# African-Robotics-Unit/AcinoSet

Measured on AMD Instinct MI355X. Metric: FTE frames/sec (residual+Jac+LM step), 6-cam x 20-joint, higher is better.
Workload: dtype f64

## Files before the change

acinoset_amd/csrc/chunk.hip:

```cpp
#include "chunk.hpp"

#include <algorithm>
#include <cstdlib>

#include "bcr_dev.hpp"
#include "trio80.hpp"

namespace acino {

void ChunkPlan::build(int nodes_total, int chunk_nodes, bool pin_l, bool pin_r) {
  n_nodes = nodes_total;
  m = n_chunks = n_sep = 0;
  node0 = pin_l ? 1 : 0;
  pin_right = pin_r ? 1 : 0;
  const int nodes = nodes_total - node0;
  if (chunk_nodes < 0 || nodes < 1) return;
  int mm = chunk_nodes;
  if (mm == 0) {
    mm = (nodes + 255) / 256;
    mm = std::max(4, std::min(mm, 512));
  }
  mm = std::max(2, mm);
  m = mm;
  n_chunks = (nodes + mm - 1) / mm;
  if (pin_r && n_chunks > 1 && nodes - (n_chunks - 1) * mm == 1) --n_chunks;
  n_sep = n_chunks - 1 + node0 + pin_right;
}

__device__ __forceinline__ d4 tile_u_ut(const double* X, int ib, int jb, int li, int lk) {
  const double* pa = X + (ib * 16 + li) * LD + ib * 16 + lk;
  const double* pb = X + (jb * 16 + li) * LD + ib * 16 + lk;
  const d4 z = {0, 0, 0, 0};
  switch (ib) {
    case 0: return mma_seq<20, false>(z, pa, 4, pb, 4);
    case 1: return mma_seq<16, false>(z, pa, 4, pb, 4);
    case 2: return mma_seq<12, false>(z, pa, 4, pb, 4);
    case 3: return mma_seq<8, false>(z, pa, 4, pb, 4);
    default: return mma_seq<4, false>(z, pa, 4, pb, 4);
  }
}
__device__ __forceinline__ void tile_store(double* M, int ib, int jb, const d4& a, int li, int lk) {
#pragma unroll
  for (int rr = 0; rr < 4; ++rr) M[(ib * 16 + lk + 4 * rr) * LD + jb * 16 + li] = a[rr];
}

constexpr int SW_VEC = 18 * NP + 2 * BS + 8 + 8 + 3 * NP + 64;
static constexpr size_t kSweepLds = (3 * MAT + SW_VEC) * sizeof(double);

__device__ __forceinline__ int opaque(int x) {
  asm volatile("" : "+v"(x));
  return x;
}

constexpr int SW_T = 512;
template <int NQ>
__device__ __forceinline__ void syrk_mask_n(d4 (&acc)[NQ], bool load) {
#pragma unroll
  for (int q = 0; q < NQ; ++q)
#pragma unroll
    for (int rr = 0; rr < 4; ++rr) acc[q][rr] = load ? acc[q][rr] : 0.0;
}
constexpr int SP_STEPS = 4 * NT - 1;
__device__ __forceinline__ void spike_gf(const double* G, const double (&bF)[NT][4], d4 (&acc)[NT], int li, int lk) {
  double a[3][NT];
  const double* gb = G + lk * LD + li;
  auto fetch = [&](int buf, int step) {
#pragma unroll
    for (int ib = 0; ib < NT; ++ib) a[buf][ib] = gb[(4 * step) * LD + ib * 16];
  };
#pragma unroll
  for (int ib = 0; ib < NT; ++ib) acc[ib] = d4{0, 0, 0, 0};
  fetch(0, 0);
  fetch(1, 1);
#pragma unroll
  for (int step = 0; step < SP_STEPS; ++step) {
    if (step + 2 < SP_STEPS) fetch((step + 2) % 3, step + 2);
    __builtin_amdgcn_sched_barrier(0);
#pragma unroll
    for (int ib = 0; ib < NT; ++ib) acc[ib] = mfma(a[step % 3][ib], bF[step >> 2][step & 3], acc[ib]);
    __builtin_amdgcn_sched_barrier(0);
  }
}
template <int NQ>
__device__ __forceinline__ void spike_ftt(d4 (&acc)[NQ], const double* Yf, const d4 (&T)[NT], const int (&as)[NQ], int li, int lk) {
  constexpr int DEPTH = NQ >= 3 ? 2 : (NQ == 2 ? 3 : 6);
  const double* p = Yf + lk * LD + li;
  double a[DEPTH + 1][NQ];
#pragma unroll
  for (int d = 0; d < DEPTH; ++d)
#pragma unroll
    for (int q = 0; q < NQ; ++q) a[d][q] = p[(4 * d) * LD + as[q] * 16];
#pragma unroll
  for (int st = 0; st < SP_STEPS; ++st) {
    if (st + DEPTH < SP_STEPS) {
#pragma unroll
      for (int q = 0; q < NQ; ++q) a[(st + DEPTH) % (DEPTH + 1)][q] = p[(4 * (st + DEPTH)) * LD + as[q] * 16];
    }
    __builtin_amdgcn_sched_barrier(0);
#pragma unroll
    for (int q = 0; q < NQ; ++q) acc[q] = mfma(-a[st % (DEPTH + 1)][q], T[st >> 2][st & 3], acc[q]);
    __builtin_amdgcn_sched_barrier(0);
  }
}
template <int NQ>
struct AlTiles {
  d4 acc[NQ];
  int as[NQ], j;
  double* Ag;
  __device__ __forceinline__ double* at(int q, int rr, int li, int lk) const {
    return as[q] >= j ? Ag + (size_t)(as[q] * 16 + 4 * rr + lk) * BS + j * 16 + li
                      : Ag + (size_t)(j * 16 + li) * BS + as[q] * 16 + 4 * rr + lk;
  }
  __device__ __forceinline__ void fetch(int li, int lk) {
#pragma unroll
    for (int q = 0; q < NQ; ++q)
#pragma unroll
      for (int rr = 0; rr < 4; ++rr) acc[q][rr] = *at(q, rr, li, lk);
  }
  __device__ __forceinline__ void run(bool load, const double* Yf, const d4 (&T)[NT], int li, int lk) {
    syrk_mask_n<NQ>(acc, load);
    spike_ftt<NQ>(acc, Yf, T, as, li, lk);
#pragma unroll
    for (int q = 0; q < NQ; ++q)
#pragma unroll
      for (int rr = 0; rr < 4; ++rr) *at(q, rr, li, lk) = acc[q][rr];
  }
};
__device__ __forceinline__ int role8(int wave) { return (0x75236410u >> (4 * wave)) & 15; }
struct GramQueue {
  int *open, *ticket, *done;
};
__device__ __forceinline__ void gram_help(const GramQueue& q, const double* Xf, double* Xg, int k, int li, int lk, int lane) {
  for (;;) {
    int t = 0;
    if (lane == 0) t = __hip_atomic_fetch_add(q.ticket, 1, __ATOMIC_RELAXED, __HIP_MEMORY_SCOPE_WORKGROUP);
    t = __builtin_amdgcn_readfirstlane(t) - 15 * k;
    if (t >= 15) {
      if (lane == 0) __hip_atomic_fetch_add(q.ticket, -1, __ATOMIC_RELAXED, __HIP_MEMORY_SCOPE_WORKGROUP);
      return;
    }
    const int ib = tri_i(t), jb = tri_j(t);
    const d4 g = tile_u_ut(Xf, ib, jb, li, lk);
#pragma unroll
    for (int rr = 0; rr < 4; ++rr) {
      Xg[(ib * 16 + lk + 4 * rr) * LD + jb * 16 + li] = g[rr];
      if (ib != jb) Xg[(jb * 16 + li) * LD + ib * 16 + lk + 4 * rr] = g[rr];
    }
    lds_signal(q.done, lane);
  }
}

struct SpikeArgs {
  const double* Xg;
  double* Y;
  double* Ag;
  const double* cRk;
  const double* bvn;
  double* zk;
  int *c_gfdone, *c_fready, *c_bv, *tdone;
  GramQueue gq;
  const double* Xf;
  int k, n_s;
  bool hasL, has_next;
  long long* stamps;
};
template <int ROLE>
__device__ __forceinline__ void spike_node(const SpikeArgs& A, int& tsb, int ln) {
  constexpr bool two = ROLE == 5;
  constexpr int j0 = ROLE == 4 ? 1 : (ROLE == 5 ? 2 : (ROLE == 6 ? 3 : 4));
  constexpr int NA = ROLE == 4 ? 3 : (ROLE == 5 ? 2 : (ROLE == 6 ? 5 : 4));
  const int li = ln & 15, lk = ln >> 4;
  double* const Y = A.Y;
  auto stamp = [&](int i) { if (A.stamps && ln == 0) A.stamps[i] = (long long)wall_clock64(); };
  AlTiles<NA> al;
  AlTiles<1> al0;
  al.Ag = A.Ag;
  al.j = j0;
  if (ROLE == 4) { al.as[0] = 1; al.as[1] = 0; al.as[2 % NA] = 2; }
  if (ROLE == 5) { al.as[0] = 2; al.as[1] = 0; }
  if (ROLE == 6) { al.as[0] = 3; al.as[1] = 0; al.as[2 % NA] = 1; al.as[3 % NA] = 2; al.as[4 % NA] = 4; }
  if (ROLE == 7) { al.as[0] = 4; al.as[1] = 0; al.as[2 % NA] = 1; al.as[3 % NA] = 2; }
  al0.Ag = A.Ag;
  al0.j = 0;
  al0.as[0] = 0;
  if (A.hasL) {
    al.fetch(li, lk);
    if (two) al0.fetch(li, lk);
  }
  lds_wait(A.gq.open, A.k + 1);
  gram_help(A.gq, A.Xf, const_cast<double*>(A.Xg), A.k, li, lk, ln);
  lds_wait(A.gq.done, 15 * (A.k + 1));
  stamp(16 + 4 * (ROLE - 4));
  d4 T0[NT], T1[NT];
  {
    double bF[NT][4];
    const double* yb = Y + lk * LD + j0 * 16 + li;
#pragma unroll
    for (int kb = 0; kb < NT; ++kb)
#pragma unroll
      for (int s = 0; s < 4; ++s) bF[kb][s] = (4 * kb + s < SP_STEPS) ? yb[(kb * 16 + 4 * s) * LD] : 0.0;
    spike_gf(A.Xg, bF, T0, li, lk);
  }
  if (two) {
    double bF[NT][4];
    const double* yb = Y + lk * LD + li;
#pragma unroll
    for (int kb = 0; kb < NT; ++kb)
#pragma unroll
      for (int s = 0; s < 4; ++s) bF[kb][s] = (4 * kb + s < SP_STEPS) ? yb[(kb * 16 + 4 * s) * LD] : 0.0;
    spike_gf(A.Xg, bF, T1, li, lk);
  }
  lds_signal(A.c_gfdone, ln);
  stamp(17 + 4 * (ROLE - 4));
  if (A.hasL) {
    lds_wait(A.c_fready, A.n_s * A.k);
    al.run(A.k > 0, Y, T0, li, lk);
    if (two) al0.run(A.k > 0, Y, T1, li, lk);
  }
  stamp(18 + 4 * (ROLE - 4));
  if (A.hasL) {
    if (ROLE != 5) lds_signal(A.tdone + (ROLE == 4 ? 0 : (ROLE == 6 ? 1 : 2)), ln);
    if (ROLE == 7 || ROLE == 4 || ROLE == 5) lds_wait(A.tdone + 1, A.k + 1);
    if (ROLE == 4 || ROLE == 5) lds_wait(A.tdone + 2, A.k + 1);
    if (ROLE == 5) lds_wait(A.tdone + 0, A.k + 1);
  }
  (void)tsb;
#pragma unroll
  for (int ib = 0; ib < NT; ++ib) tile_store(Y, ib, j0, T0[ib], li, lk);
  if (two) {
#pragma unroll
    for (int ib = 0; ib < NT; ++ib) tile_store(Y, ib, 0, T1[ib], li, lk);
  }
  if (ROLE == 7) {
    A.zk[ln] = Y[ln * LD + (BS - 1)];
    if (ln < 16) A.zk[64 + ln] = Y[(64 + ln) * LD + (BS - 1)];
  }
  if (A.has_next) {
    lds_wait(A.c_bv, A.k + 1);
    const double* const cRk = A.cRk;
    const double* const bvn = A.bvn;
    const int p = ln % NP, cg = ln / NP;
#pragma unroll
    for (int h = 0; h < (two ? 2 : 1); ++h) {
      const int c_lo = 16 * (h ? 0 : j0);
      if (cg < 2) {
        const double e00 = cRk[(0 * 3 + 0) * NP + p], e01 = cRk[(0 * 3 + 1) * NP + p], e02 = cRk[(0 * 3 + 2) * NP + p];
        const double e11 = cRk[(1 * 3 + 1) * NP + p], e12 = cRk[(1 * 3 + 2) * NP + p], e22 = cRk[(2 * 3 + 2) * NP + p];
        const double b0 = bvn[p], b1 = bvn[NP + p], b2 = bvn[2 * NP + p];
        double fv[8][3];
#pragma unroll
        for (int q = 0; q < 8; ++q) {
          const int cc = c_lo + cg + 2 * q;
          fv[q][0] = Y[p * LD + cc];
          fv[q][1] = Y[(NP + p) * LD + cc];
          fv[q][2] = Y[(2 * NP + p) * LD + cc];
        }
#pragma unroll
        for (int q = 0; q < 8; ++q) {
          const int cc = c_lo + cg + 2 * q;
          const double f0 = fv[q][0], f1 = fv[q][1], f2 = fv[q][2];
          double o0 = -(e00 * f0 + e01 * f1 + e02 * f2), o1 = -(e11 * f1 + e12 * f2), o2 = -(e22 * f2);
          if (cc == BS - 1) {
            o0 += b0;
            o1 += b1;
            o2 += b2;
          }
          Y[p * LD + cc] = o0;
          Y[(NP + p) * LD + cc] = o1;
          Y[(2 * NP + p) * LD + cc] = o2;
        }
      }
      if (ln < 16)
        for (int r = 3 * NP; r < BS; ++r) Y[r * LD + c_lo + ln] = 0.0;
    }
  }
  lds_signal(A.c_fready, ln);
  stamp(19 + 4 * (ROLE - 4));
}


__global__ void __launch_bounds__(SW_T)
k_chunk_sweep(BcrChain ch, SepView sp, const FteConst* __restrict__ cst, int* numeric_err, const int* __restrict__ status,
                int m, int n_chunks, int node0, int pin_right) {
  extern __shared__ __attribute__((aligned(16))) char smem_raw[];
  if (status && *status != 0) return;
  double* const Xf = reinterpret_cast<double*>(smem_raw);
  double* const Xg = Xf + MAT;
  double* const Y = Xg + MAT;
  double* const cL = Y + MAT;
  double* const cR0 = cL + 9 * NP;
  double* const bvb = cR0 + 9 * NP;
  double* const red = bvb + 2 * BS;
  int* const sync = reinterpret_cast<int*>(red + 8);
  int* const cB = sync + 5;
  int* const tdone = sync + 2;
  int* const g_done = sync + 6;
  int* const g_open = sync + 10;
  int* const g_ticket = sync + 1;
  int* const c_gfdone = sync + 7;
  int* const c_fready = sync + 8;
  int* const c_bv = sync + 9;
  double* const kq = red + 16;
  double* const klo = kq + NP;
  double* const khi = klo + NP;
  long long* const lst = reinterpret_cast<long long*>(khi + NP);
  const int tid = threadIdx.x, wave = tid >> 6, lane = tid & 63;
  const FteConst& K = *cst;
  const int c = blockIdx.x;
  const int first = node0 + c * m;
  const bool hasL = c > 0 || node0 > 0, hasR = c + 1 < n_chunks || pin_right;
  const int len = c + 1 < n_chunks ? m : ch.n_nodes - first;
  const int n_int = hasR ? len - 1 : len;
  const int sL = c - 1 + node0, sR = c + node0;
  const size_t MB = (size_t)BS * BS;
  const int role = __builtin_amdgcn_readfirstlane(role8(wave));
  const bool uni_tables = coupling_tables_uniform(K, first, first + n_int - 1);
  const int n_s = hasL ? 4 : 1;
  const bool builder = role <= 3;
  const bool strips = role >= 4 && (hasL || role == 7);
  double gmax_run = 0.0;
  long long* const dbgp = (ch.dbg && (long long)blockIdx.x == ch.dbg[64] && ch.dbg[66] == 0) ? ch.dbg : nullptr;
  const int dbg_k = dbgp ? (int)ch.dbg[65] : -1;
  if (dbgp && lane == 0) {
    const unsigned hw = __builtin_amdgcn_s_getreg((31 << 11) | 4);
    atomicOr(reinterpret_cast<unsigned long long*>(ch.dbg + 67), (unsigned long long)((hw >> 4) & 3) << (4 * wave));
    if (wave == 0) ch.dbg[68] = hw;
  }
#define SW_STAMP(i) do { if (dbgp && k == dbg_k && lane == 0) lst[i] = (long long)wall_clock64(); } while (0)
  if (tid < 16) sync[tid] = 0;
  if (tid < 64) lst[tid] = 0;
  if (dbgp && tid == 0) dbgp[70] = (long long)wall_clock64();
  if (c == 0 && node0) {
    for (int e = tid; e < BS * BS; e += SW_T) sp.D[e] = 0.0;
    if (tid < BS) sp.b[tid] = 0.0;
  }
  if (tid < NP) {
    kq[tid] = K.q_w[tid];
    klo[tid] = K.lo[tid];
    khi[tid] = K.hi[tid];
  }
  __syncthreads();

  TrioSync tsy;
  {
    NodeFetch f;
    build_fetch<SW_T>(f, ch, K, first, tid);
    fill_coupling_coef<SW_T>(cL, cR0, K, first, tid, kq);
    for (int e = tid; e < MAT; e += SW_T) Y[e] = 0.0;
    gmax_run = build_finish<SW_T>(Xf, bvb, f, K, first, tid, kq, klo, khi);
    __syncthreads();
    if (dbgp && tid == 0) lst[60] = (long long)wall_clock64();
    if (hasL)
      for (int e = tid; e < 9 * NP; e += SW_T) {
        const int pair = e / NP, p = e % NP, ii = pair / 3, jj = pair % 3;
        if (ii <= jj) Y[(ii * NP + p) * LD + jj * NP + p] = cL[e];
      }
    if (tid < BS) Y[tid * LD + (BS - 1)] = bvb[tid];
    __syncthreads();
    if (role < 3) chol80_trio(Xf, role, lane, numeric_err, sync, tsy);
    __syncthreads();
    if (dbgp && tid == 0) lst[61] = (long long)wall_clock64();
  }

  int tb = 0, tsb = 0;
#pragma unroll 1
  for (int k = 0; k < n_int; ++k) {
    const int node = first + k, next = node + 1;
    const bool last = k + 1 == n_int;
    const bool has_next = !last || hasR;
    const int ln = opaque(lane);
    const int li = ln & 15, lk = ln >> 4;
    double* const cRk = (uni_tables || !(k & 1)) ? cR0 : cL;
    if (builder) {
      const int bw = role;
      const int bt = bw * 64 + ln;
      const int fb_next = 3 * (next - node0);
      double hq[2][3] = {{0, 0, 0}, {0, 0, 0}}, xq[3] = {0, 0, 0}, gq[3] = {0, 0, 0}, cvq[3] = {0, 0, 0}, lamq = 0.0;
      bool liveq[3] = {false, false, false}, ownq[3] = {false, false, false};
      int pdq[2], pcq[2];
      bool ownp[2], dgp[2];
      int pdg = 0;
      bool anydg = false;
#pragma unroll
      for (int sl = 0; sl < 2; ++sl) {
        const int e = bt + 256 * sl;
        ownp[sl] = e < 13 * NP;
        const int pa = ownp[sl] ? e / 13 : 0, dd = ownp[sl] ? e % 13 : 0;
        pdq[sl] = pa;
        pcq[sl] = pa + dd >= NP ? pa + dd - NP : pa + dd;
        dgp[sl] = ownp[sl] && dd == 0;
        if (dgp[sl]) pdg = pa;
        anydg = anydg || dgp[sl];
      }
      if (has_next) {
        const int cur = ch.st->cur;
        const double* Hg = cur ? ch.H1 : ch.H0;
        lamq = ch.st->lam;
#pragma unroll
        for (int j = 0; j < 3; ++j)
          if (fb_next + j < K.n_frames) {
#pragma unroll
            for (int sl = 0; sl < 2; ++sl)
              if (ownp[sl]) hq[sl][j] = Hg[(size_t)(fb_next + j) * HPAIRS + bt + 256 * sl];
          }
        if (anydg) {
          const double* xg = cur ? ch.x1 : ch.x0;
          const double* gg = cur ? ch.g1 : ch.g0;
#pragma unroll
          for (int j = 0; j < 3; ++j)
            if (fb_next + j < K.n_frames) {
              xq[j] = xg[(size_t)(fb_next + j + HALO) * NP + pdg];
              gq[j] = gg[(size_t)(fb_next + j) * NP + pdg];
            }
#pragma unroll
          for (int pr = 0; pr < 3; ++pr) {
            const int j = pr == 2 ? 1 : 0, jp = pr == 0 ? 1 : 2;
            if (fb_next + jp < K.n_frames)
              cvq[pr] = 2.0 * kq[pdg] * band_coef_clip(K.n_offset + fb_next + j, jp - j, K.n_global, K.clip_len);
          }
        }
#pragma unroll
        for (int j = 0; j < 3; ++j) {
          liveq[j] = fb_next + j < K.n_frames;
          ownq[j] = fb_next + j >= K.own_lo && fb_next + j < K.own_hi;
        }
      }
      if (bw == 0) SW_STAMP(0);
      lds_barrier(cB, tb, 4, ln);
      lds_wait(c_gfdone, n_s * k);
      if (bw == 0) SW_STAMP(1);
      const GramQueue gqu{g_open, g_ticket, g_done};
      if (bt == 0) __hip_atomic_fetch_add(g_open, 1, __ATOMIC_RELAXED, __HIP_MEMORY_SCOPE_WORKGROUP);
      if (k > 0 && !uni_tables) fill_coupling_coef<256>(nullptr, cRk, K, node, bt, kq);
      gram_help(gqu, Xf, Xg, k, li, lk, ln);
      SW_STAMP(32 + wave);
      lds_barrier(cB, tb, 4, ln);
      lds_wait(g_done, 15 * (k + 1));
      if (bw == 0) SW_STAMP(2);
#pragma unroll
      for (int j = 0; j < 3; ++j) asm volatile("" : "+v"(hq[0][j]), "+v"(hq[1][j]), "+v"(xq[j]), "+v"(gq[j]));
      asm volatile("" : "+v"(lamq));
      if (has_next) {
        double* const bvn = bvb + ((k + 1) & 1) * BS;
        double ca[2][6], cb[2][6], gv[2][3][3];
#pragma unroll
        for (int sl = 0; sl < 2; ++sl) {
          const int pr = pdq[sl], pc = pcq[sl];
          ca[sl][0] = cRk[0 * NP + pr]; ca[sl][1] = cRk[1 * NP + pr]; ca[sl][2] = cRk[2 * NP + pr];
          ca[sl][3] = cRk[4 * NP + pr]; ca[sl][4] = cRk[5 * NP + pr]; ca[sl][5] = cRk[8 * NP + pr];
          cb[sl][0] = cRk[0 * NP + pc]; cb[sl][1] = cRk[1 * NP + pc]; cb[sl][2] = cRk[2 * NP + pc];
          cb[sl][3] = cRk[4 * NP + pc]; cb[sl][4] = cRk[5 * NP + pc]; cb[sl][5] = cRk[8 * NP + pc];
#pragma unroll
          for (int jj = 0; jj < 3; ++jj) {
            const double* gp = Xg + (jj * NP + pr) * LD + pc;
            gv[sl][jj][0] = gp[0];
            gv[sl][jj][1] = gp[NP];
            gv[sl][jj][2] = gp[2 * NP];
          }
        }
#pragma unroll
        for (int sl = 0; sl < 2; ++sl) {
          const int pr = pdq[sl], pc = pcq[sl];
          const bool dg = dgp[sl];
          const double a00 = ca[sl][0], a01 = ca[sl][1], a02 = ca[sl][2], a11 = ca[sl][3], a12 = ca[sl][4], a22 = ca[sl][5];
          const double b00 = cb[sl][0], b01 = cb[sl][1], b02 = cb[sl][2], b11 = cb[sl][3], b12 = cb[sl][4], b22 = cb[sl][5];
          double mm[3][3], S[3][3];
#pragma unroll
          for (int jj = 0; jj < 3; ++jj) {
            const double g0 = gv[sl][jj][0], g1 = gv[sl][jj][1], g2 = gv[sl][jj][2];
            mm[jj][0] = g0 * b00 + g1 * b01 + g2 * b02;
            mm[jj][1] = g1 * b11 + g2 * b12;
            mm[jj][2] = g2 * b22;
          }
#pragma unroll
          for (int ii = 0; ii < 3; ++ii) {
            S[0][ii] = a00 * mm[0][ii] + a01 * mm[1][ii] + a02 * mm[2][ii];
            S[1][ii] = a11 * mm[1][ii] + a12 * mm[2][ii];
            S[2][ii] = a22 * mm[2][ii];
          }
          double v[3][3];
#pragma unroll
          for (int j = 0; j < 3; ++j)
#pragma unroll
            for (int jp = 0; jp < 3; ++jp) v[j][jp] = (j == jp ? hq[sl][j] : 0.0);
          if (dg) {
#pragma unroll
            for (int j = 0; j < 3; ++j) {
              double d = 1.0, bb = 0.0;
              if (liveq[j]) {
                d = hq[sl][j];
                const double gtol = GRAD_ZERO_REL * d;
                const bool fixed = (xq[j] <= klo[pr] && gq[j] > gtol) || (xq[j] >= khi[pr] && gq[j] < -gtol);
                d = d + lamq * fmax(d, DIAG_FLOOR);
                if (fixed) d *= FIX_SCALE;
                bb = fixed ? 0.0 : -gq[j];
                if (ownq[j]) gmax_run = fmax(gmax_run, fabs(bb));
              }
              v[j][j] = d;
              bvn[j * NP + pr] = bb;
            }
            v[0][1] = v[1][0] = cvq[0];
            v[0][2] = v[2][0] = cvq[1];
            v[1][2] = v[2][1] = cvq[2];
          }
          if (ownp[sl]) {
#pragma unroll
            for (int j = 0; j < 3; ++j)
#pragma unroll
              for (int jp = 0; jp < 3; ++jp) {
                const double val = v[j][jp] - S[j][jp];
                Xf[(j * NP + pr) * LD + jp * NP + pc] = val;
                if (!dg) Xf[(jp * NP + pc) * LD + j * NP + pr] = val;
              }
          }
        }
        if (bt < BS - 3 * NP) {
          Xf[(3 * NP + bt) * LD + 3 * NP + bt] = 1.0;
          bvn[3 * NP + bt] = 0.0;
        }
      }
      lds_barrier(cB, tb, 4, ln);
      if (bt == 0) __hip_atomic_fetch_add(c_bv, 1, __ATOMIC_RELAXED, __HIP_MEMORY_SCOPE_WORKGROUP);
      if (bw == 0) SW_STAMP(4);
      if (bw < 3) {
        if (!last) chol80_trio<false>(Xf, bw, ln, numeric_err, sync, tsy, (dbgp && k == dbg_k) ? lst : nullptr);
        SW_STAMP(8 + wave);
      } else if (bw == 3) {
        double* Gg = ch.D + node * MB;
#pragma unroll 6
        for (int q = 0; q < LOWER_ITEMS / 64; ++q) {
          const int idx = ln + 64 * q;
          int r, cc;
          lower_item(idx, r, cc);
          *reinterpret_cast<double2*>(Gg + r * BS + cc) = make_double2(Xg[r * LD + cc], Xg[r * LD + cc + 1]);
        }
        SW_STAMP(8 + wave);
      }
    }
    if (strips) {
      SpikeArgs sa;
      sa.Xg = Xg; sa.Y = Y; sa.Ag = sp.AL + (size_t)(hasL ? opaque(sL) : 0) * MB; sa.cRk = cRk; sa.bvn = bvb + ((k + 1) & 1) * BS;
      sa.zk = ch.b + (size_t)node * BS; sa.gq = GramQueue{g_open, g_ticket, g_done}; sa.Xf = Xf; sa.c_gfdone = c_gfdone; sa.c_fready = c_fready; sa.c_bv = c_bv; sa.tdone = tdone;
      sa.k = k; sa.n_s = n_s; sa.hasL = hasL; sa.has_next = has_next; sa.stamps = (dbgp && k == dbg_k) ? lst : nullptr;
      if (role == 4) spike_node<4>(sa, tsb, ln);
      else if (role == 5) spike_node<5>(sa, tsb, ln);
      else if (role == 6) spike_node<6>(sa, tsb, ln);
      else spike_node<7>(sa, tsb, ln);
    }
  }
  __syncthreads();
  if (dbgp) {
    if (tid == 0) lst[62] = (long long)wall_clock64();
    __syncthreads();
    if (tid < 64 && lst[tid]) dbgp[tid] = lst[tid];
  }
  if (hasR) {
    {
      double2* d2 = reinterpret_cast<double2*>(sp.D + (size_t)sR * MB);
      for (int idx = tid; idx < BS * BS / 2; idx += SW_T) {
        const int e = 2 * idx, r = e / BS, cc = e % BS;
        d2[idx] = make_double2(Xf[r * LD + cc], Xf[r * LD + cc + 1]);
      }
    }
    if (tid < BS) sp.b[(size_t)sR * BS + tid] = Y[tid * LD + (BS - 1)];
    if (hasL) {
      double* Cg = sp.Cpl + (size_t)sL * MB;
      for (int e = tid; e < BS * BS; e += SW_T) {
        const int r = e / BS, cc = e % BS;
        Cg[e] = cc < 3 * NP ? Y[r * LD + cc] : 0.0;
      }
    }
  }
#undef SW_STAMP
  publish_gmax<SW_T>(gmax_run, red, ch.gn_part, c, tid);
  if (dbgp && tid == 0) dbgp[71] = (long long)wall_clock64();
}

__global__ void __launch_bounds__(256) k_sep_combine(SepView sp, const int* __restrict__ status) {
  if (status && *status != 0) return;
  const int q = blockIdx.x, tid = threadIdx.x;
  const size_t MB = (size_t)BS * BS;
  double* D = sp.D + q * MB;
  const double* A = sp.AL + q * MB;
  constexpr int NQ = (LOWER_ITEMS + 255) / 256;
  double2 dv[NQ], av[NQ];
  const double bq = tid < 3 * NP ? sp.b[(size_t)q * BS + tid] : 0.0, aq = tid < 3 * NP ? A[(size_t)(BS - 1) * BS + tid] : 0.0;
#pragma unroll
  for (int k = 0; k < NQ; ++k) {
    const int idx = tid + 256 * k;
    if (idx < LOWER_ITEMS) {
      int r, cc;
      lower_item(idx, r, cc);
      dv[k] = *reinterpret_cast<const double2*>(D + r * BS + cc);
      av[k] = *reinterpret_cast<const double2*>(A + r * BS + cc);
    }
  }
#pragma unroll
  for (int k = 0; k < NQ; ++k) {
    const int idx = tid + 256 * k;
    if (idx < LOWER_ITEMS) {
      int r, cc;
      lower_item(idx, r, cc);
      if (r < 3 * NP) {
        const double ax = cc < 3 * NP ? av[k].x : 0.0, ay = cc + 1 < 3 * NP ? av[k].y : 0.0;
        *reinterpret_cast<double2*>(D + r * BS + cc) = make_double2(dv[k].x + ax, dv[k].y + ay);
      }
    }
  }
  if (tid < 3 * NP) sp.b[(size_t)q * BS + tid] = bq + aq;
}

constexpr int BK_PW = 4;
constexpr int BK_NL = 4;
constexpr int BK_T = 64 * (BK_PW + BK_NL);
constexpr int BK_NB = 2;
constexpr int BLD = 82;
constexpr int BK_Q = LOWER_ITEMS / 64;
constexpr int BK_FL = 8;
static_assert(LOWER_ITEMS == 64 * NT * (NT + 1), "30 rounds of 64 items: 2 (ib + 1) per tile row");
static_assert(BK_FL >= BK_NL + BK_NB + 2, "a far f_k must have been stored (and waited for) before a loader asks for it");
constexpr int BK_OPS = BS * BLD, BK_TAB = BK_OPS + 5 * BS, BK_STAGE = BK_TAB + 9 * NP + 1;
static constexpr size_t kBacksubLds =
    (BK_NB * BK_STAGE + 2 * BS + BK_FL * BS + 2 * 9 * NP + 16 + NP + 1) * sizeof(double) + 16 * sizeof(int);

typedef double d2 __attribute__((ext_vector_type(2)));
template <int CTRL>
__device__ __forceinline__ double dpp_add(double v) {
  const long long b = __double_as_longlong(v);
  const int lo = __builtin_amdgcn_update_dpp(0, (int)b, CTRL, 0xf, 0xf, false);
  const int hi = __builtin_amdgcn_update_dpp(0, (int)(b >> 32), CTRL, 0xf, 0xf, false);
  return v + __longlong_as_double(((long long)hi << 32) | (unsigned)lo);
}
__device__ __forceinline__ double lanes8_sum(double v) {
  v = dpp_add<0x141>(v);
  v = dpp_add<0xB1>(v);
  return dpp_add<0x4E>(v);
}
__global__ void __launch_bounds__(BK_T)
k_chunk_backsub(BcrChain ch, SepView sp, const FteConst* __restrict__ cst, const int* __restrict__ status, int m,
                int n_chunks, int node0, int pin_right, TrialOut trial) {
  extern __shared__ __attribute__((aligned(16))) char smem_raw[];
  double* const stg = reinterpret_cast<double*>(smem_raw);
  double* const ub = stg + BK_NB * BK_STAGE;
  double* const fl = ub + 2 * BS;
  double* const cL0 = fl + BK_FL * BS;
  double* const cRl = cL0 + 9 * NP;
  double* const red = cRl + 9 * NP;
  double* const kq = red + 16;
  int* const sync = reinterpret_cast<int*>(kq + NP + 1);
  int* const c_ready = sync;
  int* const c_rd = sync + BK_NL;
  int* const c_u = sync + BK_NL + 1;
  const int tid = threadIdx.x, lane = tid & 63, wave = tid >> 6;
  const int c = blockIdx.x, first = node0 + c * m;
  const bool hasL = c > 0 || node0 > 0, hasR = c + 1 < n_chunks || pin_right;
  const int len = c + 1 < n_chunks ? m : ch.n_nodes - first;
  const int n_int = hasR ? len - 1 : len;
  const int sL = c - 1 + node0, sR = c + node0;
  const size_t MB = (size_t)BS * BS;
  const int nf = hasL && n_int > 0 ? n_int - 1 : 0;
  const int ns = nf + n_int;
  auto node_at = [&](int s) __attribute__((always_inline)) { return s < nf ? s : n_int - 1 - (s - nf); };
  struct Rounds {
    int row0[BK_Q], col0[BK_Q];
    constexpr Rounds() : row0{}, col0{} {
      int q = 0;
      for (int ib = 0; ib < NT; ++ib)
        for (int h = 0; h < 2; ++h)
          for (int jc = 0; jc <= ib; ++jc) {
            row0[q] = 16 * ib + 8 * h;
            col0[q] = 16 * jc;
            ++q;
          }
    }
  };
  constexpr Rounds RD{};
  const int gl = (lane >> 3) * BS + 2 * (lane & 7), ll = (lane >> 3) * BLD + 2 * (lane & 7);
  d2 g[BK_Q];
  const int gl74 = ((lane >> 3) < 3 ? (lane >> 3) : 2) * BS + 2 * (lane & 7);
  auto tile_fetch = [&](int k) __attribute__((always_inline)) {
    const double* G = ch.D + (size_t)(first + k) * MB;
#pragma unroll
    for (int q = 0; q < BK_Q; ++q)
      g[q] = *reinterpret_cast<const d2*>(G + (RD.row0[q] * BS + RD.col0[q]) + (RD.row0[q] + 8 > 3 * NP ? gl74 : gl));
  };
  const int lw = wave - BK_PW;
  if (lw >= 0 && lw < ns) tile_fetch(node_at(lw));
  if (status && *status != 0) return;
  const FteConst& K = *cst;
  const bool uni = coupling_tables_uniform(K, first, first + n_int - 1);
  auto table_node = [&](int s) __attribute__((always_inline)) {
    const int k = node_at(s);
    return s < nf ? k : (k > 0 ? k - 1 : 0);
  };
  const int t_cur = ch.st->cur, t_nf = K.n_frames;
  const double* t_x = t_cur ? ch.x1 : ch.x0;
  const double* t_g = t_cur ? ch.g1 : ch.g0;
  const double* t_hd = t_cur ? trial.hd1 : trial.hd0;
  double* const fst = ch.Wl + (size_t)first * BS;
  if (ch.dbg && (long long)blockIdx.x == ch.dbg[64] && ch.dbg[66] == 1 && tid == 0) ch.dbg[61] = (long long)wall_clock64();
  if (c == 0 && sp.flags) {
    for (int e = tid; e < sp.n_flags; e += BK_T) sp.flags[e] = 0;
    if (tid == 0) sp.flags[sp.n_flags] += 1;
  }
  if (tid < 16) sync[tid] = 0;
  if (tid < 2 * BS) ub[tid] = 0.0;
  if (tid < NP) kq[tid] = K.q_w[tid];
  fill_coupling_coef<BK_T>(cL0, nullptr, K, first, tid);
  fill_coupling_coef<BK_T>(nullptr, cRl, K, first + (n_int > 0 ? n_int - 1 : 0), tid);
  double t_pred = 0.0, t_step = 0.0;
  if (wave >= BK_PW) {
    constexpr int NRO = (5 * 3 * NP + 63) / 64;
    double ro[NRO];
    auto ro_fetch = [&](int t) __attribute__((always_inline)) {
      if (t < nf) return;
      const int k = node_at(t), node = first + k;
      const bool far = hasL && k >= 1 && n_int - k >= BK_FL;
      const int ln = opaque(lane);
#pragma unroll
      for (int j = 0; j < NRO; ++j) {
        const int e = ln + 64 * j < 5 * 3 * NP ? ln + 64 * j : 5 * 3 * NP - 1, o = e / (3 * NP), r = e % (3 * NP);
        int n = 3 * (node - node0) + r / NP;
        n = n < t_nf ? n : t_nf - 1;
        const size_t nr = (size_t)n * NP + r % NP;
        const double* src = o == 0 ? ch.b + (size_t)node * BS + r
                          : o == 1 ? t_x + nr + (size_t)HALO * NP
                          : o == 2 ? t_g + nr
                          : o == 3 ? t_hd + nr
                                   : fst + (size_t)(far ? k - 1 : 0) * BS + r;
        ro[j] = *src;
      }
      if (lane < BS - 3 * NP) ch.b[(size_t)node * BS + 3 * NP + lane] = 0.0;
    };
    if (lw < ns) ro_fetch(lw);
    __syncthreads();
    for (int t = lw; t < ns; t += BK_NL) {
      const bool bwd = t >= nf;
      long long* const ldbg = (ch.dbg && (long long)blockIdx.x == ch.dbg[64] && ch.dbg[66] == 1 && lane == 0 && t >= 10 && t < 14) ? ch.dbg + 48 + 4 * (t - 10) : nullptr;
      if (ldbg) ldbg[0] = (long long)wall_clock64();
      if (t >= BK_NB) lds_wait(c_rd, BK_PW * (t - BK_NB + 1));
      if (ldbg) { __builtin_amdgcn_s_waitcnt(0x0F70); ldbg[1] = (long long)wall_clock64(); }
      double* const St = stg + (t % BK_NB) * BK_STAGE;
#pragma unroll
      for (int q = 0; q < BK_Q; ++q) *reinterpret_cast<d2*>(St + ll + (RD.row0[q] * BLD + RD.col0[q])) = g[q];
      if (bwd) {
        const int ln = opaque(lane);
#pragma unroll
        for (int j = 0; j < NRO; ++j) {
          const int e = ln + 64 * j;
          if (e < 5 * 3 * NP) St[BK_OPS + (e / (3 * NP)) * BS + e % (3 * NP)] = ro[j];
        }
      }
      if (uni) {
        if (t < BK_NB) right_table_interior<64>(St + BK_TAB, lane, [&](int p) { return kq[p]; });
      } else if (right_table_is_interior(K, first + table_node(t))) {
        right_table_interior<64>(St + BK_TAB, lane, [&](int p) { return kq[p]; });
      } else {
        fill_coupling_coef<64>(nullptr, St + BK_TAB, K, first + table_node(t), lane, kq);
      }
      if (ldbg) { __builtin_amdgcn_s_waitcnt(0xC07F); ldbg[2] = (long long)wall_clock64(); }
      lds_signal(c_ready + lw, lane);
      if (t + BK_NL < ns) {
        tile_fetch(node_at(t + BK_NL));
        ro_fetch(t + BK_NL);
      }
    }
  } else {
    const int pg = lane >> 3, part = lane & 7;
    const int p = 8 * wave + pg, pc = p < NP ? p : NP - 1;
    const int a = part < 3 ? part : 2, ra = a * NP + pc;
    const bool rowl = p < NP && part < 3;
    const int t_own_lo = K.own_lo, t_own_hi = K.own_hi;
    const double t_lam = ch.st->lam;
    double* t_xt = const_cast<double*>(t_cur ? ch.x0 : ch.x1);
    const double t_lo = K.lo[pc], t_hi = K.hi[pc];
    auto trial_row = [&](int node, double delta, double xv, double gv, double d0) __attribute__((always_inline)) {
      const int n = 3 * (node - node0) + a;
      if (rowl && n < t_nf) {
        const double gtol = GRAD_ZERO_REL * d0;
        const bool fixed = (xv <= t_lo && gv > gtol) || (xv >= t_hi && gv < -gtol);
        const double d = fixed ? 0.0 : delta, pg_ = fixed ? 0.0 : gv;
        const double xnew = fmin(fmax(xv + d, t_lo), t_hi);
        t_xt[(size_t)(n + HALO) * NP + pc] = xnew;
        if (n >= t_own_lo && n < t_own_hi) {
          t_pred += 0.5 * d * (t_lam * fmax(d0, DIAG_FLOOR) * d - pg_);
          t_step = fmax(t_step, fabs(xnew - xv));
        }
      }
    };
    constexpr int NJ = BS / 8;
    int gdir[3], gtrn[3], gtile[3];
#pragma unroll
    for (int aa = 0; aa < 3; ++aa) {
      const int r = aa * NP + pc;
      gdir[aa] = r * BLD + part;
      gtrn[aa] = part * BLD + r;
      gtile[aa] = r >> 4;
    }
    double xr[3] = {0, 0, 0}, xl[3] = {0, 0, 0};
    if (hasR) {
#pragma unroll
      for (int ii = 0; ii < 3; ++ii) xr[ii] = sp.b[(size_t)sR * BS + ii * NP + pc];
      if (tid < BS) ch.b[(size_t)(first + n_int) * BS + tid] = sp.b[(size_t)sR * BS + tid];
    }
    if (hasL) {
#pragma unroll
      for (int jj = 0; jj < 3; ++jj) xl[jj] = sp.b[(size_t)sL * BS + jj * NP + pc];
    }
    double s_xv, s_gv, s_d0;
    {
      int n = 3 * (first + n_int - node0) + a;
      n = n < t_nf ? n : t_nf - 1;
      s_xv = t_x[(size_t)(n + HALO) * NP + pc];
      s_gv = t_g[(size_t)n * NP + pc];
      s_d0 = t_hd[(size_t)n * NP + pc];
    }
    __syncthreads();
    double wR = 0.0, f0 = 0.0;
#pragma unroll
    for (int ii = 0; ii < 3; ++ii)
      if (ii <= a) wR += cRl[(ii * 3 + a) * NP + pc] * xr[ii];
#pragma unroll
    for (int jj = 0; jj < 3; ++jj)
      if (jj >= a) f0 += cL0[(a * 3 + jj) * NP + pc] * xl[jj];
    if (rowl) {
      ub[ra] = nf > 0 ? f0 : f0 + wR;
      if (hasL) {
        fst[ra] = f0;
        fl[ra] = f0;
      }
    }
    lds_signal(c_u, lane);
    long long* const bdbg = (ch.dbg && (long long)blockIdx.x == ch.dbg[64] && ch.dbg[66] == 1 && tid == 0) ? ch.dbg : nullptr;
    if (bdbg) bdbg[62] = (long long)wall_clock64();
    double cf[6] = {0, 0, 0, 0, 0, 0};
    bool pend = false;
    int p_node = 0;
    double p_xa = 0.0, p_xv = 0.0, p_gv = 0.0, p_d0 = 0.0;
#pragma unroll 1
    for (int s = 0; s < ns; ++s) {
      const int b = s & 1;
      const bool fwd = s < nf;
      const int k = node_at(s), node = first + k;
      const double* const St = stg + (s % BK_NB) * BK_STAGE;
#define BK_STAMP(i) do { if (bdbg && s >= 8 && s < 16) { __builtin_amdgcn_s_waitcnt(0xC07F); bdbg[6 * (s - 8) + (i)] = (long long)wall_clock64(); } } while (0)
      lds_wait2(c_ready + (s % BK_NL), s / BK_NL + 1, c_u, BK_PW * (s + 1));
      BK_STAMP(0);
      BK_STAMP(1);
      double uv[NJ], gv[3][NJ];
#pragma unroll
      for (int j = 0; j < NJ; ++j) uv[j] = ub[b * BS + part + 8 * j];
#pragma unroll
      for (int aa = 0; aa < 3; ++aa) {
        const int gd = opaque(gdir[aa]), gt = opaque(gtrn[aa]);
#pragma unroll
        for (int j = 0; j < NJ; ++j) gv[aa][j] = St[(j >> 1) <= gtile[aa] ? gd + 8 * j : gt + 8 * j * BLD];
      }
      if (!uni || s < BK_NB) {
        const double* T = St + BK_TAB;
        cf[0] = T[0 * NP + pc]; cf[1] = T[1 * NP + pc]; cf[2] = T[2 * NP + pc];
        cf[3] = T[4 * NP + pc]; cf[4] = T[5 * NP + pc]; cf[5] = T[8 * NP + pc];
      }
      const double z0 = St[BK_OPS + pc], z1 = St[BK_OPS + NP + pc], z2 = St[BK_OPS + 2 * NP + pc];
      const double o_xv = St[BK_OPS + BS + ra], o_gv = St[BK_OPS + 2 * BS + ra], o_d0 = St[BK_OPS + 3 * BS + ra];
      const double o_f = St[BK_OPS + 4 * BS + ra];
      const double fnear = fl[((k > 0 ? k - 1 : 0) % BK_FL) * BS + ra];
      lds_signal(c_rd, lane);
      if (pend) {
        if (rowl) ch.b[(size_t)p_node * BS + ra] = p_xa;
        trial_row(p_node, p_xa, p_xv, p_gv, p_d0);
        pend = false;
      }
      BK_STAMP(2);
      double y[3];
#pragma unroll
      for (int aa = 0; aa < 3; ++aa) {
        double v0 = gv[aa][0] * uv[0], v1 = gv[aa][1] * uv[1];
#pragma unroll
        for (int j = 2; j < NJ; j += 2) {
          v0 = fma(gv[aa][j], uv[j], v0);
          v1 = fma(gv[aa][j + 1], uv[j + 1], v1);
        }
        y[aa] = lanes8_sum(v0 + v1);
      }
      if (bdbg && s >= 8 && s < 16) { asm volatile("" :: "v"(y[0]), "v"(y[1]), "v"(y[2])); bdbg[6 * (s - 8) + 3] = (long long)wall_clock64(); }
      if (fwd) {
        const double f0_ = -(cf[0] * y[0] + cf[1] * y[1] + cf[2] * y[2]);
        const double f1_ = -(cf[3] * y[1] + cf[4] * y[2]);
        const double f2_ = -(cf[5] * y[2]);
        const double fn = a == 0 ? f0_ : (a == 1 ? f1_ : f2_);
        if (rowl) {
          ub[(b ^ 1) * BS + ra] = s + 1 == nf ? fn + wR : fn;
          fl[((k + 1) % BK_FL) * BS + ra] = fn;
          fst[(size_t)(k + 1) * BS + ra] = fn;
        }
        if (s + 1 == nf) __builtin_amdgcn_s_waitcnt(0x0F70);
        lds_signal(c_u, lane);
        BK_STAMP(4);
      } else {
        const double x0 = z0 - y[0], x1 = z1 - y[1], x2 = z2 - y[2];
        const double xa = a == 0 ? x0 : (a == 1 ? x1 : x2);
        const double e0 = cf[0] * x0, e1 = cf[1] * x0 + cf[3] * x1, e2 = cf[2] * x0 + cf[4] * x1 + cf[5] * x2;
        const double fk = hasL ? (n_int - k < BK_FL ? fnear : o_f) : 0.0;
        if (rowl && k > 0) ub[(b ^ 1) * BS + ra] = fk + (a == 0 ? e0 : (a == 1 ? e1 : e2));
        lds_signal(c_u, lane);
        BK_STAMP(4);
        pend = true;
        p_node = node;
        p_xa = xa;
        p_xv = o_xv;
        p_gv = o_gv;
        p_d0 = o_d0;
      }
      if (bdbg && s >= 8 && s < 16) bdbg[6 * (s - 8) + 5] = (long long)wall_clock64();
    }
#undef BK_STAMP
    if (pend) {
      if (rowl) ch.b[(size_t)p_node * BS + ra] = p_xa;
      trial_row(p_node, p_xa, p_xv, p_gv, p_d0);
    }
    if (bdbg) bdbg[63] = (long long)wall_clock64();
    if (hasR) trial_row(first + n_int, a == 0 ? xr[0] : (a == 1 ? xr[1] : xr[2]), s_xv, s_gv, s_d0);
  }
  for (int off = 32; off > 0; off >>= 1) {
    t_pred += __shfl_down(t_pred, off, 64);
    t_step = fmax(t_step, __shfl_down(t_step, off, 64));
  }
  if (lane == 0 && wave < BK_PW) {
    red[2 * wave] = t_pred;
    red[2 * wave + 1] = t_step;
  }
  __syncthreads();
  if (tid == 0) {
    double sp_ = 0.0, sm = 0.0;
#pragma unroll
    for (int w = 0; w < BK_PW; ++w) {
      sp_ += red[2 * w];
      sm = fmax(sm, red[2 * w + 1]);
    }
    trial.pred_part[c] = sp_;
    trial.step_part[c] = sm;
  }
}

int chunk_set_func_attributes() {
  ACINO_HIP_CHECK(hipFuncSetAttribute(reinterpret_cast<const void*>(k_chunk_sweep),
                                      hipFuncAttributeMaxDynamicSharedMemorySize, (int)kSweepLds));
  ACINO_HIP_CHECK(hipFuncSetAttribute(reinterpret_cast<const void*>(k_chunk_backsub),
                                      hipFuncAttributeMaxDynamicSharedMemorySize, (int)kBacksubLds));
  return ACINO_OK;
}

int chunk_reduce(const BcrChain& ch, const ChunkPlan& pl, const SepView& sp, const BcrChain& sepch,
                 const BcrSchedule& sepsch, const FteConst* d_c, int* d_numeric_err, const int* d_status, hipStream_t s,
                 Profiler* prof) {
  {
    ProfSpan span(prof, PC_CHUNK_SWEEP, s, pl.n_nodes - pl.n_sep);
    hipLaunchKernelGGL(k_chunk_sweep, dim3(pl.n_chunks), dim3(SW_T), kSweepLds, s, ch, sp, d_c, d_numeric_err, d_status, pl.m,
                       pl.n_chunks, pl.node0, pl.pin_right);
  }
  ACINO_LAUNCH_CHECK();
  if (pl.n_sep == 0) return ACINO_OK;
  if (!sepsch.consumers_add_al) {
    {
      ProfSpan span(prof, PC_SEP_COMBINE, s, pl.n_sep);
      hipLaunchKernelGGL(k_sep_combine, dim3(pl.n_sep), dim3(256), 0, s, sp, d_status);
    }
    ACINO_LAUNCH_CHECK();
  }
  return bcr_reduce(sepch, sepsch, d_c, d_numeric_err, d_status, s, prof);
}

int chunk_backsub(const BcrChain& ch, const ChunkPlan& pl, const SepView& sp, const BcrChain& sepch,
                  const BcrSchedule& sepsch, const FteConst* d_c, int* d_numeric_err, const int* d_status, hipStream_t s,
                  Profiler* prof, const TrialOut& trial) {
  if (pl.n_sep > 0) {
    int rc = bcr_backsub(sepch, sepsch, d_c, d_status, s, prof, d_numeric_err);
    if (rc) return rc;
  }
  {
    ProfSpan span(prof, PC_CHUNK_BACKSUB, s, pl.n_nodes - pl.n_sep);
    hipLaunchKernelGGL(k_chunk_backsub, dim3(pl.n_chunks), dim3(BK_T), kBacksubLds, s, ch, sp, d_c, d_status, pl.m, pl.n_chunks, pl.node0,
                       pl.pin_right, trial);
  }
  ACINO_LAUNCH_CHECK();
  return ACINO_OK;
}

}
```

Before: 23.86 million.

## Store backsub tiles in packed swizzled 16x16 LDS layout and reuse turnaround stages

Replaces the padded row-major (stride 82) LDS staging of the lower-triangular block with packed 16x16 tiles whose column pairs are XOR-swizzled, so writes and row/transposed reads avoid bank conflicts. It also raises the number of staging buffers from 2 to 4 and maps backward-sweep steps onto stages so that the first few backward nodes reuse tiles still resident from the forward sweep, skipping those global fetches and LDS writes. The cost is more LDS per block, which may lower occupancy, plus more complex stage-index and wait logic that must stay consistent between loader and solver waves.

```diff
diff --git a/acinoset_amd/csrc/chunk.hip b/acinoset_amd/csrc/chunk.hip
--- a/acinoset_amd/csrc/chunk.hip
+++ b/acinoset_amd/csrc/chunk.hip
@@ -613,13 +613,15 @@
 constexpr int BK_PW = 4;
 constexpr int BK_NL = 4;
 constexpr int BK_T = 64 * (BK_PW + BK_NL);
-constexpr int BK_NB = 2;
-constexpr int BLD = 82;
+constexpr int BK_NB = 4;
+constexpr int BK_TS = 16 * 16;
 constexpr int BK_Q = LOWER_ITEMS / 64;
-constexpr int BK_FL = 8;
+constexpr int BK_FL = 10;
 static_assert(LOWER_ITEMS == 64 * NT * (NT + 1), "30 rounds of 64 items: 2 (ib + 1) per tile row");
 static_assert(BK_FL >= BK_NL + BK_NB + 2, "a far f_k must have been stored (and waited for) before a loader asks for it");
-constexpr int BK_OPS = BS * BLD, BK_TAB = BK_OPS + 5 * BS, BK_STAGE = BK_TAB + 9 * NP + 1;
+constexpr int BK_OPS = (NT * (NT + 1) / 2) * BK_TS, BK_TAB = BK_OPS + 5 * BS, BK_STAGE = BK_TAB + 9 * NP + 1;
+static_assert(BK_STAGE % 2 == 0, "stages start on 16 bytes (ds_write_b128)");
+__host__ __device__ constexpr int bk_swz(int i) { return (((i >> 1) & 1) << 2) | (((i >> 2) & 1) << 1); }
 static constexpr size_t kBacksubLds =
     (BK_NB * BK_STAGE + 2 * BS + BK_FL * BS + 2 * 9 * NP + 16 + NP + 1) * sizeof(double) + 16 * sizeof(int);
 
@@ -661,21 +663,24 @@
   const int nf = hasL && n_int > 0 ? n_int - 1 : 0;
   const int ns = nf + n_int;
   auto node_at = [&](int s) __attribute__((always_inline)) { return s < nf ? s : n_int - 1 - (s - nf); };
+  auto stage_of = [&](int s) __attribute__((always_inline)) { return s < nf ? s % BK_NB : (nf + (BK_NB - 1) * (s - nf)) % BK_NB; };
+  auto bk_reuse = [&](int s) __attribute__((always_inline)) { return s > nf && s - nf < BK_NB && s - nf <= nf; };
   struct Rounds {
-    int row0[BK_Q], col0[BK_Q];
-    constexpr Rounds() : row0{}, col0{} {
+    int row0[BK_Q], col0[BK_Q], lds0[BK_Q];
+    constexpr Rounds() : row0{}, col0{}, lds0{} {
       int q = 0;
       for (int ib = 0; ib < NT; ++ib)
         for (int h = 0; h < 2; ++h)
           for (int jc = 0; jc <= ib; ++jc) {
             row0[q] = 16 * ib + 8 * h;
             col0[q] = 16 * jc;
+            lds0[q] = (ib * (ib + 1) / 2 + jc) * BK_TS + 8 * h * 16;
             ++q;
           }
     }
   };
   constexpr Rounds RD{};
-  const int gl = (lane >> 3) * BS + 2 * (lane & 7), ll = (lane >> 3) * BLD + 2 * (lane & 7);
+  const int gl = (lane >> 3) * BS + 2 * (lane & 7), ll = (lane >> 3) * 16 + 2 * ((lane & 7) ^ bk_swz(lane >> 3));
   d2 g[BK_Q];
   const int gl74 = ((lane >> 3) < 3 ? (lane >> 3) : 2) * BS + 2 * (lane & 7);
   auto tile_fetch = [&](int k) __attribute__((always_inline)) {
@@ -685,7 +690,7 @@
       g[q] = *reinterpret_cast<const d2*>(G + (RD.row0[q] * BS + RD.col0[q]) + (RD.row0[q] + 8 > 3 * NP ? gl74 : gl));
   };
   const int lw = wave - BK_PW;
-  if (lw >= 0 && lw < ns) tile_fetch(node_at(lw));
+  if (lw >= 0 && lw < ns && !bk_reuse(lw)) tile_fetch(node_at(lw));
   if (status && *status != 0) return;
   const FteConst& K = *cst;
   const bool uni = coupling_tables_uniform(K, first, first + n_int - 1);
@@ -738,11 +743,15 @@
       const bool bwd = t >= nf;
       long long* const ldbg = (ch.dbg && (long long)blockIdx.x == ch.dbg[64] && ch.dbg[66] == 1 && lane == 0 && t >= 10 && t < 14) ? ch.dbg + 48 + 4 * (t - 10) : nullptr;
       if (ldbg) ldbg[0] = (long long)wall_clock64();
-      if (t >= BK_NB) lds_wait(c_rd, BK_PW * (t - BK_NB + 1));
+      const bool kept = bk_reuse(t);
+      const int prev = kept ? 2 * nf - t : t - BK_NB;
+      if (prev >= 0) lds_wait(c_rd, BK_PW * (prev + 1));
       if (ldbg) { __builtin_amdgcn_s_waitcnt(0x0F70); ldbg[1] = (long long)wall_clock64(); }
-      double* const St = stg + (t % BK_NB) * BK_STAGE;
-#pragma unroll
-      for (int q = 0; q < BK_Q; ++q) *reinterpret_cast<d2*>(St + ll + (RD.row0[q] * BLD + RD.col0[q])) = g[q];
+      double* const St = stg + stage_of(t) * BK_STAGE;
+      if (!kept) {
+#pragma unroll
+        for (int q = 0; q < BK_Q; ++q) *reinterpret_cast<d2*>(St + ll + RD.lds0[q]) = g[q];
+      }
       if (bwd) {
         const int ln = opaque(lane);
 #pragma unroll
@@ -761,7 +770,7 @@
       if (ldbg) { __builtin_amdgcn_s_waitcnt(0xC07F); ldbg[2] = (long long)wall_clock64(); }
       lds_signal(c_ready + lw, lane);
       if (t + BK_NL < ns) {
-        tile_fetch(node_at(t + BK_NL));
+        if (!bk_reuse(t + BK_NL)) tile_fetch(node_at(t + BK_NL));
         ro_fetch(t + BK_NL);
       }
     }
@@ -789,13 +798,14 @@
       }
     };
     constexpr int NJ = BS / 8;
-    int gdir[3], gtrn[3], gtile[3];
+    int gdir[3], gdir1[3], gtrn[3], gtile[3];
 #pragma unroll
     for (int aa = 0; aa < 3; ++aa) {
-      const int r = aa * NP + pc;
-      gdir[aa] = r * BLD + part;
-      gtrn[aa] = part * BLD + r;
-      gtile[aa] = r >> 4;
+      const int r = aa * NP + pc, ib = r >> 4, i = r & 15;
+      gdir[aa] = (ib * (ib + 1) / 2) * BK_TS + i * 16 + 2 * ((part >> 1) ^ bk_swz(i)) + (part & 1);
+      gdir1[aa] = gdir[aa] ^ 8;
+      gtrn[aa] = ib * BK_TS + part * 16 + 2 * ((i >> 1) ^ bk_swz(part)) + (i & 1);
+      gtile[aa] = ib;
     }
     double xr[3] = {0, 0, 0}, xl[3] = {0, 0, 0};
     if (hasR) {
@@ -842,7 +852,7 @@
       const int b = s & 1;
       const bool fwd = s < nf;
       const int k = node_at(s), node = first + k;
-      const double* const St = stg + (s % BK_NB) * BK_STAGE;
+      const double* const St = stg + stage_of(s) * BK_STAGE;
 #define BK_STAMP(i) do { if (bdbg && s >= 8 && s < 16) { __builtin_amdgcn_s_waitcnt(0xC07F); bdbg[6 * (s - 8) + (i)] = (long long)wall_clock64(); } } while (0)
       lds_wait2(c_ready + (s % BK_NL), s / BK_NL + 1, c_u, BK_PW * (s + 1));
       BK_STAMP(0);
@@ -852,9 +862,11 @@
       for (int j = 0; j < NJ; ++j) uv[j] = ub[b * BS + part + 8 * j];
 #pragma unroll
       for (int aa = 0; aa < 3; ++aa) {
-        const int gd = opaque(gdir[aa]), gt = opaque(gtrn[aa]);
-#pragma unroll
-        for (int j = 0; j < NJ; ++j) gv[aa][j] = St[(j >> 1) <= gtile[aa] ? gd + 8 * j : gt + 8 * j * BLD];
+        const int gd = opaque(gdir[aa]), gd1 = opaque(gdir1[aa]), gt = opaque(gtrn[aa]);
+#pragma unroll
+        for (int j = 0; j < NJ; ++j)
+          gv[aa][j] = St[(j >> 1) <= gtile[aa] ? ((j & 1) ? gd1 : gd) + (j >> 1) * BK_TS
+                                               : gt + ((j >> 1) * ((j >> 1) + 1) / 2) * BK_TS + (j & 1) * 8 * 16];
       }
       if (!uni || s < BK_NB) {
         const double* T = St + BK_TAB;
```

Result: no change. 23.74 million (-0.5%).
